# kaspanet/rusty-kaspa

Hardware: NVIDIA H100
Metric: schnorr_sig_verifies_per_sec (higher is better)
Workload: dtype u32 limbs (256-bit modular integer)

## Files before the change

__graft_entry__.py:

```python
import os
import subprocess
import sys

ROOT = os.path.dirname(os.path.abspath(__file__))
CSRC = os.path.join(ROOT, "rusty_kaspa_b200", "csrc")
LIB = os.path.join(ROOT, "rusty_kaspa_b200", "libkgv.so")
NVCC_FLAGS = ["-gencode", "arch=compute_90a,code=sm_90a", "-O3", "-lineinfo", "-std=c++17", "-shared", "-Xcompiler", "-fPIC"]


def _newer(target, sources):
    if not os.path.exists(target):
        return True
    t = os.path.getmtime(target)
    return any(os.path.getmtime(s) > t for s in sources)


def _run(cmd, **kw):
    r = subprocess.run(cmd, capture_output=True, text=True, **kw)
    if r.returncode != 0:
        raise RuntimeError("command failed: %s\n%s\n%s" % (" ".join(cmd), r.stdout[-4000:], r.stderr[-4000:]))
    return r


def build():
    srcs = [os.path.join(d, f) for d, _, fs in os.walk(CSRC) for f in fs] + [os.path.join(ROOT, "include", "kgv.h")]
    units = sorted(s for s in srcs if s.endswith(".cu") or s.endswith(".cpp"))
    if _newer(LIB, srcs):
        nvcc = os.environ.get("NVCC", "nvcc")
        _run([nvcc] + NVCC_FLAGS + ["-o", LIB] + units)
    _run(["make", "-C", os.path.join(ROOT, "oracle")])
    hs = os.path.join(ROOT, "tests", "hostsim")
    for name in ("hostsim_arith", "hostsim_secp", "hostsim_comb", "hostsim_joint", "hostsim_joint_record", "hostsim_hash", "hostsim_u3072", "hostsim_script", "hostsim_standard", "hostsim_chain", "hostsim_pow"):
        src, out = os.path.join(hs, name + ".cpp"), os.path.join(hs, "lib" + name + ".so")
        if os.path.exists(src) and _newer(out, [src] + srcs):
            _run(["g++", "-O2", "-std=c++17", "-shared", "-fPIC", "-o", out, src])
    op_src, op_lib = os.path.join(ROOT, "tests", "oracle_pow", "ok_pow.c"), os.path.join(ROOT, "tests", "oracle_pow", "libok_pow.so")
    if _newer(op_lib, [op_src]):
        _run(["gcc", "-O2", "-std=c11", "-fPIC", "-shared", "-pthread", "-o", op_lib, op_src, "-lm"])
    sg_src, sg_lib = os.path.join(ROOT, "tools", "simgen", "kgv_simgen.cpp"), os.path.join(ROOT, "tools", "simgen", "libkgv_simgen.so")
    if os.path.exists(sg_src) and _newer(sg_lib, [sg_src]):
        _run(["g++", "-O2", "-std=c++17", "-shared", "-fPIC", "-o", sg_lib, sg_src])
    for name in ("host_mirror_test", "script_engine_mirror_test"):
        cpp_src, cpp_bin = os.path.join(ROOT, "tests", "cpp", name + ".cpp"), os.path.join(ROOT, "tests", "cpp", name)
        if os.path.exists(cpp_src) and _newer(cpp_bin, [cpp_src, LIB, os.path.join(ROOT, "include", "kgv.hpp"), os.path.join(ROOT, "include", "kgv.h")]):
            _run(["g++", "-O2", "-std=c++17", "-o", cpp_bin, cpp_src, "-L" + os.path.join(ROOT, "rusty_kaspa_b200"), "-l:libkgv.so", "-Wl,-rpath,$ORIGIN/../../rusty_kaspa_b200"])
    sys.path.insert(0, ROOT)
    import rusty_kaspa_b200
    from rusty_kaspa_b200 import _lib
    _lib.load()


def smoke():
    import ctypes
    import numpy as np
    sys.path.insert(0, ROOT)
# ... 56 lines not shown
```

rusty_kaspa_b200/csrc/kgv_internal.h:

```cpp
#pragma once
#include <cuda_runtime.h>
#include <cstdint>
#include <condition_variable>
#include <cstdio>
#include <initializer_list>
#include <memory>
#include <mutex>
#include <string>
#include <thread>
#include <vector>

#ifndef KGV_BLOCK
#define KGV_BLOCK 128
#endif
#ifndef KGV_BLOCKS_PER_SM
#define KGV_BLOCKS_PER_SM 3
#endif

#ifndef KGV_ITEMS
#define KGV_ITEMS 4
#endif

struct kgv_ctx {
  int device = 0;
  cudaStream_t own_stream = nullptr;
  cudaStream_t aux_stream = nullptr;
  cudaEvent_t ev_fork = nullptr, ev_join = nullptr;
  cudaEvent_t ev_time[3] = {};
  cudaEvent_t ev_chunk[32] = {};
  cudaStream_t stream = nullptr;
  uint32_t* gtab = nullptr;
  uint8_t* d_io = nullptr;
  size_t d_io_cap = 0;
  uint8_t* d_in = nullptr;
  size_t d_in_cap = 0;
  uint8_t* d_out = nullptr;
  size_t d_out_cap = 0;
  uint8_t* d_batch = nullptr;
  size_t d_batch_cap = 0;
  struct PrefetchSlot {
// ... 204 lines not shown
```

rusty_kaspa_b200/csrc/kgv_lib.cu:

```cuda
#include "../../include/kgv.h"
#include "kgv_internal.h"
#include "kgv_verify.cuh"
#include "kgv_lanes.cuh"

#include <cuda_runtime.h>
#include <cstdio>
#include <algorithm>
#include <cstring>
#include <mutex>
#include <string>

using namespace kgv;

struct SmemTab {
  uint32_t* base;
  __device__ __forceinline__ void put(int e, int w, uint32_t v) { base[(e * 16 + w) * KGV_BLOCK] = v; }
  __device__ __forceinline__ uint32_t get(int e, int w) const { return base[(e * 16 + w) * KGV_BLOCK]; }
  __device__ __forceinline__ uint4* chunk(int q) const { return reinterpret_cast<uint4*>(base - threadIdx.x) + q * KGV_BLOCK + threadIdx.x; }
};
__device__ __forceinline__ void stage_fetch(SmemTab& tab, int s, const uint32_t* entry) {
#pragma unroll
  for (int c = 0; c < 4; c++) {
    const uint32_t dst = (uint32_t)__cvta_generic_to_shared(tab.chunk(4 * s + c));
    asm volatile("cp.async.cg.shared.global [%0], [%1], 16;" ::"r"(dst), "l"(entry + 4 * c) : "memory");
  }
}
__device__ __forceinline__ void stage_commit(SmemTab&) { asm volatile("cp.async.commit_group;" ::: "memory"); }
__device__ __forceinline__ void stage_wait(SmemTab&) { asm volatile("cp.async.wait_group 7;" ::: "memory"); }
__device__ __forceinline__ void stage_get(SmemTab& tab, int s, fe& x, fe& y) {
  const uint4 a = *tab.chunk(4 * s), b = *tab.chunk(4 * s + 1), c = *tab.chunk(4 * s + 2), d = *tab.chunk(4 * s + 3);
  x.v[0] = a.x; x.v[1] = a.y; x.v[2] = a.z; x.v[3] = a.w; x.v[4] = b.x; x.v[5] = b.y; x.v[6] = b.z; x.v[7] = b.w;
  y.v[0] = c.x; y.v[1] = c.y; y.v[2] = c.z; y.v[3] = c.w; y.v[4] = d.x; y.v[5] = d.y; y.v[6] = d.z; y.v[7] = d.w;
}

__device__ __forceinline__ void ldg256(uint32_t* w, const void* p) {
  asm volatile("ld.global.nc.v4.u32 {%0,%1,%2,%3}, [%8];\n\t"
               "ld.global.nc.v4.u32 {%4,%5,%6,%7}, [%8+16];"
               : "=r"(w[0]), "=r"(w[1]), "=r"(w[2]), "=r"(w[3]), "=r"(w[4]), "=r"(w[5]), "=r"(w[6]), "=r"(w[7])
               : "l"(p));
}
__device__ __forceinline__ void ldg256_stream(uint32_t* w, const void* p) {
  asm volatile("ld.global.nc.L1::no_allocate.v4.u32 {%0,%1,%2,%3}, [%8];\n\t"
               "ld.global.nc.L1::no_allocate.v4.u32 {%4,%5,%6,%7}, [%8+16];"
               : "=r"(w[0]), "=r"(w[1]), "=r"(w[2]), "=r"(w[3]), "=r"(w[4]), "=r"(w[5]), "=r"(w[6]), "=r"(w[7])
               : "l"(p));
}

struct GLoadDev {
  __device__ __forceinline__ void operator()(fe& x, fe& y, const uint32_t* entry) const {
    ldg256(x.v, entry);
    ldg256(y.v, entry + 8);
  }
};

template <bool ALIGNED>
__device__ __forceinline__ void load_be32(uint32_t* w, const uint8_t* p) {
  if (ALIGNED) {
    ldg256_stream(w, p);
#pragma unroll
    for (int i = 0; i < 8; i++) w[i] = bswap32(w[i]);
  } else {
#pragma unroll
    for (int i = 0; i < 8; i++)
      w[i] = ((uint32_t)p[4 * i] << 24) | ((uint32_t)p[4 * i + 1] << 16) | ((uint32_t)p[4 * i + 2] << 8) | (uint32_t)p[4 * i + 3];
  }
}

__global__ void __launch_bounds__(128) k_build_gtab(uint32_t* __restrict__ gtab) {
  uint32_t t = blockIdx.x * blockDim.x + threadIdx.x;
  if (t >= 8u * 65536u) return;
  uint32_t v = t & 0xFFFFu;
  uint32_t which = t >> 16;
  uint32_t* out = gtab + (size_t)t * 16;
  if (v == 0) {
#pragma unroll
    for (int i = 0; i < 16; i++) out[i] = 0;
    return;
  }
  fe bx, by, x, y;
  gtab_base(bx, by, (int)which);
  gtab_entry(x, y, v, bx, by);
#pragma unroll
  for (int i = 0; i < 8; i++) { out[i] = x.v[i]; out[8 + i] = y.v[i]; }
}

#define KGV_KEY_RECORDS_MAX (1u << 17)
#ifndef KGV_COMB_USES
#define KGV_COMB_USES 8
#endif
enum { KGV_KEYS_INLINE = 0, KGV_KEYS_PLAIN = 1, KGV_KEYS_COMB = 2 };
__host__ __device__ __forceinline__ int key_form(uint32_t n_rec, size_t n) {
  if (n_rec > KGV_KEY_RECORDS_MAX || 2 * (size_t)n_rec > n) return KGV_KEYS_INLINE;
  return (size_t)KGV_COMB_USES * n_rec <= n ? KGV_KEYS_COMB : KGV_KEYS_PLAIN;
}

struct KeySlot {
  unsigned long long key;
  uint32_t rec, unused_;
};
struct KeyCacheView {
  const KeySlot* table;
  const uint32_t* item_slot;
  const uint32_t* recs;
  const uint32_t* n_rec;
  const uint32_t* item_rec;
  const uint32_t* kc_recs;
// ... 481 lines not shown
  if (rc) return rc;
  *cap = want;
  return KGV_OK;
}

extern "C" int kgv_create(int device, uint32_t flags, kgv_ctx** out) {
  (void)flags;
  if (!out) return KGV_ERR_ARG;
  *out = nullptr;
  int ndev = 0;
  if (cudaGetDeviceCount(&ndev) != cudaSuccess || ndev <= 0 || device < 0 || device >= ndev) {
    (void)cudaGetLastError();
    return KGV_ERR_CUDA;
  }
  kgv_ctx* ctx = new kgv_ctx();
  ctx->device = device;
  auto body = [&]() -> int {
    CK(cudaSetDevice(device));
    CK(cudaStreamCreateWithFlags(&ctx->own_stream, cudaStreamNonBlocking));
    ctx->stream = ctx->own_stream;
    CK(cudaStreamCreateWithFlags(&ctx->aux_stream, cudaStreamNonBlocking));
    CK(cudaEventCreateWithFlags(&ctx->ev_fork, cudaEventDisableTiming));
    CK(cudaEventCreateWithFlags(&ctx->ev_join, cudaEventDisableTiming));
    CK(cudaMalloc((void**)&ctx->gtab, (size_t)8 * 65536 * 16 * sizeof(uint32_t)));
    k_build_gtab<<<(8 * 65536) / 128, 128, 0, ctx->stream>>>(ctx->gtab);
    CK(cudaGetLastError());
    ctx->launches++;
    const int smem = KGV_BLOCK * 128 * (int)sizeof(uint32_t);
    for (const auto& kind : k_verify)
      for (const auto& form : kind)
        for (VerifyKernel k : form) CK(cudaFuncSetAttribute(k, cudaFuncAttributeMaxDynamicSharedMemorySize, smem));
    int per_sm = 0, sms = 0;
    CK(cudaOccupancyMaxActiveBlocksPerMultiprocessor(&per_sm, k_verify[0][0][1], KGV_BLOCK, smem));
    CK(cudaDeviceGetAttribute(&sms, cudaDevAttrMultiProcessorCount, device));
    ctx->resident_blocks = per_sm * sms > 0 ? per_sm * sms : 132 * KGV_BLOCKS_PER_SM;
    CK(cudaStreamSynchronize(ctx->stream));
    return KGV_OK;
  };
  int rc = body();
  if (rc != KGV_OK) {
    fprintf(stderr, "kgv_create: %s\n", ctx->err.c_str());
    delete ctx;
    return rc;
  }
  *out = ctx;
  return KGV_OK;
}

extern "C" void kgv_destroy(kgv_ctx* ctx) {
  if (!ctx) return;
  cudaSetDevice(ctx->device);
// ... 146 lines not shown
    P.stamp = 2;
  }
  CK(cudaMemsetAsync(S, 0, 256, st));
  return KGV_OK;
}
static int kc_insert(kgv_ctx* ctx, kgv_keycache::Part& P, const KcScratch& s, size_t n, bool ecdsa, cudaStream_t st, bool gate) {
  CK(cudaMemsetAsync(s.table, 0, (size_t)s.slots * sizeof(KeySlot), st));
  const uint32_t slots = P.v.n_sets * KGV_KC_WAYS, limit = gate ? std::min(slots, (uint32_t)KGV_KEY_RECORDS_MAX) : 0xFFFFFFFFu;
  const auto dedup = ecdsa ? k_key_dedup<false, true, true> : k_key_dedup<true, false, true>;
  dedup<<<nblk(n, 256), 256, 0, st>>>(s.miss_keys, n, nullptr, s.hdr + KC_N_MISS, s.table, s.slots - 1, s.item_slot, s.rec_rep, s.hdr + KC_N_REC,
                                      limit);
  CK(cudaGetLastError());
  const auto insert = ecdsa ? k_kc_insert<true> : k_kc_insert<false>;
  insert<<<nblk(n, KGV_BLOCK), KGV_BLOCK, 0, st>>>(P.v, s.miss_keys, s.rec_rep, s.hdr, P.stamp, gate);
  CK(cudaGetLastError());
  ctx->launches += 2;
  return KGV_OK;
}

int kgv_launch_verify(kgv_ctx* ctx, const uint8_t* dpk, const uint8_t* dmsg, const uint8_t* dsig, size_t n, uint8_t* dst, bool ecdsa,
                      cudaStream_t st, const uint32_t* index, const uint32_t* n_dev) {
  if (n == 0) return KGV_OK;
  if (n >= 0x7FFFFFFFu) return fail_arg(ctx, "verify launch of 2^31 or more items");
  const int smem = KGV_BLOCK * 128 * (int)sizeof(uint32_t);
  size_t want = (n + KGV_BLOCK - 1) / KGV_BLOCK;
  unsigned blocks = (unsigned)(want < (size_t)ctx->resident_blocks ? want : (size_t)ctx->resident_blocks);
  bool aligned = (((uintptr_t)dmsg | (uintptr_t)dsig | (ecdsa ? 0 : (uintptr_t)dpk)) & 31) == 0;
  KeyCacheView kc{};
  const bool key_cache = n > (size_t)ctx->resident_blocks * KGV_BLOCK;
  kgv_keycache::Part* kp = ctx->keycache && ctx->keycache->enabled && ctx->keycache->part[ecdsa].v.n_sets ? &ctx->keycache->part[ecdsa] : nullptr;
  if (!index) {
    auto& lv = ctx->last_verify[ecdsa];
    lv.n = n; lv.blocks = blocks; lv.key_cache = key_cache && !kp; lv.stream = st;
  }
  if (!kp) {
    if (key_cache) {
      int rc = key_cache_launch(ctx, dpk, n, ecdsa, aligned, st, index, n_dev, &kc);
      if (rc) return rc;
    }
    k_verify[ecdsa][index != nullptr][aligned]<<<blocks, KGV_BLOCK, smem, st>>>(dpk, dmsg, dsig, n, dst, ctx->gtab, index, n_dev, kc);
    CK(cudaGetLastError());
    ctx->launches++;
    return KGV_OK;
  }
  KcScratch ks{};
  if (int rc = kc_begin(ctx, *kp, n, ecdsa, st, &ks)) return rc;
  const auto lookup = ecdsa ? k_kc_lookup<false, true> : aligned ? k_kc_lookup<true, false> : k_kc_lookup<false, false>;
// ... 188 lines not shown
  io.out(bitmap, nbytes, &ddst);
  if (int rc = io.stage()) return rc;
  k_status_to_bitmap<<<(unsigned)((nbytes + 255) / 256), 256, 0, ctx->stream>>>(dsrc, n, ddst);
  CK(cudaGetLastError());
  ctx->launches++;
  return io.finish();
}

extern "C" int kgv_debug_schnorr_trace(kgv_ctx* ctx, const uint8_t* pk32, const uint8_t* msg32, const uint8_t* sig64, uint32_t* trace_words,
                                       uint8_t* status) {
  if (!ctx) return KGV_ERR_ARG;
  std::lock_guard<std::recursive_mutex> g(ctx->mu);
  if (!pk32 || !msg32 || !sig64 || !trace_words || !status) return fail_arg(ctx, "null buffer");
  CK(cudaSetDevice(ctx->device));
  const size_t tw = KGV_TRACE_STAGES * 16 * sizeof(uint32_t);
  int rc = kgv_reserve(ctx, &ctx->d_in, &ctx->d_in_cap, 256);
  if (rc) return rc;
  rc = kgv_reserve(ctx, &ctx->d_out, &ctx->d_out_cap, tw + 256);
  if (rc) return rc;
  CK(cudaMemcpyAsync(ctx->d_in, pk32, 32, cudaMemcpyHostToDevice, ctx->stream));
  CK(cudaMemcpyAsync(ctx->d_in + 32, msg32, 32, cudaMemcpyHostToDevice, ctx->stream));
  CK(cudaMemcpyAsync(ctx->d_in + 64, sig64, 64, cudaMemcpyHostToDevice, ctx->stream));
  CK(cudaMemsetAsync(ctx->d_out, 0, tw + 256, ctx->stream));
  const int smem = KGV_BLOCK * 128 * (int)sizeof(uint32_t);
  CK(cudaFuncSetAttribute(k_schnorr_trace, cudaFuncAttributeMaxDynamicSharedMemorySize, smem));
  k_schnorr_trace<<<1, KGV_BLOCK, smem, ctx->stream>>>(ctx->d_in, ctx->d_in + 32, ctx->d_in + 64, ctx->d_out + tw, ctx->gtab, (uint32_t*)ctx->d_out);
  CK(cudaGetLastError());
  ctx->launches++;
  CK(cudaMemcpyAsync(trace_words, ctx->d_out, tw, cudaMemcpyDeviceToHost, ctx->stream));
  CK(cudaMemcpyAsync(status, ctx->d_out + tw, 1, cudaMemcpyDeviceToHost, ctx->stream));
  CK(cudaStreamSynchronize(ctx->stream));
  return KGV_OK;
}

extern "C" int kgv_debug_key_form(kgv_ctx* ctx, int ecdsa, kgv_key_form_info* out) {
  if (!ctx) return KGV_ERR_ARG;
  std::lock_guard<std::recursive_mutex> g(ctx->mu);
  if (!out) return fail_arg(ctx, "null buffer");
  const auto& lv = ctx->last_verify[ecdsa ? 1 : 0];
  if (lv.n == 0) return fail_arg(ctx, "no verify launch of that kind yet");
  CK(cudaSetDevice(ctx->device));
  CK(cudaStreamSynchronize(lv.stream));
  uint32_t n_rec = 0;
  if (lv.key_cache) CK(cudaMemcpy(&n_rec, ctx->d_keys[ecdsa ? 1 : 0], sizeof n_rec, cudaMemcpyDeviceToHost));
  out->n_items = lv.n;
  out->threads = (uint64_t)lv.blocks * KGV_BLOCK;
  out->distinct_keys = n_rec;
// ... 9 lines not shown
  if (!ctx) return KGV_ERR_ARG;
  std::lock_guard<std::recursive_mutex> g(ctx->mu);
  if (!in_words || !out_words || n == 0 || n > (1u << 20)) return fail_arg(ctx, "bad selftest arguments");
  CK(cudaSetDevice(ctx->device));
  int rc = kgv_reserve(ctx, &ctx->d_in, &ctx->d_in_cap, n * 64);
  if (rc) return rc;
  rc = kgv_reserve(ctx, &ctx->d_out, &ctx->d_out_cap, n * 64);
  if (rc) return rc;
  CK(cudaMemcpyAsync(ctx->d_in, in_words, n * 64, cudaMemcpyHostToDevice, ctx->stream));
  if (op >= 12)
    k_selftest_lanes<<<(unsigned)((n * 8 + 63) / 64), 64, 0, ctx->stream>>>(op, (const uint32_t*)ctx->d_in, (uint32_t*)ctx->d_out, (int)n);
  else
    k_selftest<<<(unsigned)((n + 63) / 64), 64, 0, ctx->stream>>>(op, (const uint32_t*)ctx->d_in, (uint32_t*)ctx->d_out, (int)n);
  CK(cudaGetLastError());
  ctx->launches++;
  CK(cudaMemcpyAsync(out_words, ctx->d_out, n * 64, cudaMemcpyDeviceToHost, ctx->stream));
  CK(cudaStreamSynchronize(ctx->stream));
  return KGV_OK;
}

extern "C" int kgv_gtable_entry(kgv_ctx* ctx, int which, uint32_t v, uint8_t out_xy[64]) {
  if (!ctx) return KGV_ERR_ARG;
  std::lock_guard<std::recursive_mutex> g(ctx->mu);
  if ((which != 0 && which != 1) || v == 0 || v > 65535 || !out_xy) return fail_arg(ctx, "bad table index");
  CK(cudaSetDevice(ctx->device));
  uint32_t w[16];
  CK(cudaMemcpyAsync(w, ctx->gtab + ((size_t)which * 4 * 65536 + v) * 16, sizeof w, cudaMemcpyDeviceToHost, ctx->stream));
  CK(cudaStreamSynchronize(ctx->stream));
  for (int c = 0; c < 2; c++)
    for (int i = 0; i < 8; i++) {
      uint32_t limb = w[c * 8 + 7 - i];
      out_xy[c * 32 + 4 * i] = (uint8_t)(limb >> 24);
      out_xy[c * 32 + 4 * i + 1] = (uint8_t)(limb >> 16);
      out_xy[c * 32 + 4 * i + 2] = (uint8_t)(limb >> 8);
      out_xy[c * 32 + 4 * i + 3] = (uint8_t)limb;
    }
  return KGV_OK;
}
```

rusty_kaspa_b200/csrc/kgv_secp.cuh:

```cuda
#pragma once
#include "kgv_arith.cuh"

namespace kgv {

#define KGV_N_LIMBS {0xD0364141u, 0xBFD25E8Cu, 0xAF48A03Bu, 0xBAAEDCE6u, 0xFFFFFFFEu, 0xFFFFFFFFu, 0xFFFFFFFFu, 0xFFFFFFFFu}
#define KGV_BETA_LIMBS {0x719501EEu, 0xC1396C28u, 0x12F58995u, 0x9CF04975u, 0xAC3434E9u, 0x6E64479Eu, 0x657C0710u, 0x7AE96A2Bu}
#define KGV_G1_LIMBS {0x45DBB031u, 0xE893209Au, 0x71E8CA7Fu, 0x3DAA8A14u, 0x9284EB15u, 0xE86C90E4u, 0xA7D46BCDu, 0x3086D221u}
#define KGV_G2_LIMBS {0x8AC47F71u, 0x1571B4AEu, 0x9DF506C6u, 0x221208ACu, 0x0ABFE4C4u, 0x6F547FA9u, 0x010E8828u, 0xE4437ED6u}
#define KGV_A1_LIMBS {0x9284EB15u, 0xE86C90E4u, 0xA7D46BCDu, 0x3086D221u, 0u}
#define KGV_MB1_LIMBS {0x0ABFE4C3u, 0x6F547FA9u, 0x010E8828u, 0xE4437ED6u, 0u}
#define KGV_A2_LIMBS {0x9D44CFD8u, 0x57C1108Du, 0xA8E2F3F6u, 0x14CA50F7u, 1u}

struct gej {
  fe x, y, z;
  bool inf;
};

struct NoTrace {
  KGV_HD void operator()(int , const uint32_t* , int ) const {}
};

KGV_HD bool sc_ge_n(const uint32_t* a) {
  const uint32_t n[8] = KGV_N_LIMBS;
  return !lt8(a, n);
// ... 338 lines not shown
  if (gej_add_ge_body(r, bx, by, hout)) {
    if (hout) fe_dbl(*hout, r.y);
    gej_double_n(r, 1);
  }
}
#endif
KGV_HD void gej_double(gej& r) { gej_double_n(r, 1); }

KGV_HD bool ge_lift_x(fe& y, const fe& x, bool odd) {
  fe t, c;
  fe_sqr(t, x);
  fe_mul(t, t, x);
  fe_set_u32(c, 7);
  fe_add(c, t, c);
  if (!fe_sqrt(y, c)) return false;
  fe_normalize(y);
  if (((y.v[0] & 1u) != 0) != odd) {
    fe_neg(y, y);
    fe_normalize(y);
  }
  return true;
}

template <int NE = 8, class Tab>
KGV_HD void build_odd_table(Tab& tab, fe& zs, const fe& px, const fe& py) {
  static_assert(NE >= 2 && NE <= 8, "build_odd_table: 2 to 8 entries");
  gej d;
  d.x = px; d.y = py; fe_set_u32(d.z, 1); d.inf = false;
  gej_double(d);
  fe zd2, zd3;
  fe_sqr(zd2, d.z);
  fe_mul(zd3, zd2, d.z);
  gej t;
  fe_mul(t.x, px, zd2);
  fe_mul(t.y, py, zd3);
  fe_set_u32(t.z, 1);
  t.inf = false;
  fe H[NE - 1];
#pragma unroll
  for (int w = 0; w < 8; w++) { tab.put(0, w, t.x.v[w]); tab.put(0, 8 + w, t.y.v[w]); }
#pragma unroll
  for (int j = 1; j < NE; j++) {
    gej_add_ge(t, d.x, d.y, &H[j - 1]);
#pragma unroll
    for (int w = 0; w < 8; w++) { tab.put(j, w, t.x.v[w]); tab.put(j, 8 + w, t.y.v[w]); }
  }
// ... 143 lines not shown
      stage_commit(tab);
    }
    if ((w & 3) == 0) {
#pragma unroll 1
      for (int j = 0; j < 8; j++) {
        const uint32_t d = (kG[j] >> (w ? 16 : 0)) & 0xFFFFu;
        if (d) {
          gload(ex, ey, gtab + ((size_t)j * 65536 + d) * 16);
          gej_add_ge(R, ex, ey);
        }
      }
    }
  }
#pragma unroll 1
  for (int half = 0; half < 2; half++) {
    if (!fix[half]) continue;
    gload(ex, ey, rec);
    if (half) fe_mul(ex, ex, beta);
    if (!ng[half]) fe_neg(ey, ey);
    gej_add_ge(R, ex, ey);
  }
}

KGV_HD void recode_joint(uint32_t* h, bool& fix, const uint32_t* m) {
  fix = (m[0] & 1u) == 0;
  uint64_t v[4], carry = fix ? 1 : 0;
#pragma unroll
  for (int t = 0; t < 3; t++) {
    const uint64_t x = (uint64_t)m[t] + carry;
    const uint32_t lo = (uint32_t)x, hi = (uint32_t)(x >> 32);
    const uint32_t borrow = ((m[t + 1] + hi) & 1u) ^ 1u;
    v[t] = (uint64_t)(lo >> 1) + (borrow ? (1ull << 31) : (1ull << 32));
    carry = hi + borrow;
  }
  const uint64_t c3 = (uint64_t)m[3] + ((uint64_t)m[4] << 32) + carry;
  v[3] = (c3 >> 1) + (1ull << 32);
#pragma unroll
  for (int q = 0; q < 5; q++) h[q] = 0;
#pragma unroll
  for (int i = 0; i < 44; i++) h[i / 10] |= (uint32_t)((v[i / 11] >> (3 * (i % 11))) & 7u) << (3 * (i % 10));
}
KGV_HD uint32_t joint_digit(const uint32_t* h, int i) { return (h[i / 10] >> (3 * (i % 10))) & 7u; }
KGV_HD const uint32_t* joint_entry(const uint32_t* jt, const uint32_t (*h)[5], const bool* ng, int i, bool& neg) {
  const uint32_t u0 = joint_digit(h[0], i), u1 = joint_digit(h[1], i);
  neg = (u0 < 4u) != ng[0];
  const uint32_t a = u0 < 4u ? 3u - u0 : u0 - 4u;
  const uint32_t k = neg != ng[1] ? 7u - u1 : u1;
  return jt + 16 * (32 * (i / 11) + 8 * a + k);
}
template <class GLoad>
KGV_HD void gen_fields(gej& R, const uint32_t* kG, int sh, const uint32_t* gtab, GLoad gload) {
  fe ex, ey;
#pragma unroll 1
  for (int j = 0; j < 8; j++) {
    const uint32_t d = (kG[j] >> sh) & 0xFFFFu;
    if (d) {
      gload(ex, ey, gtab + ((size_t)j * 65536 + d) * 16);
      gej_add_ge(R, ex, ey);
    }
  }
}
template <class Tab, class GLoad>
KGV_HD void ecmult_joint(gej& R, const uint32_t* kP, const uint32_t* kG, const uint32_t* rec, const uint32_t* jt, Tab& tab, const uint32_t* gtab,
                         GLoad gload) {
  const fe beta = {KGV_BETA_LIMBS};
  uint32_t m[2][5], h[2][5];
  bool ng[2], fix[2], neg;
  glv_split(m[0], ng[0], m[1], ng[1], kP);
  recode_joint(h[0], fix[0], m[0]);
  recode_joint(h[1], fix[1], m[1]);
#pragma unroll 1
  for (int s = 0; s < 8; s++) {
    const int w = 9 - (s >> 2), t = s & 3;
    stage_fetch(tab, 4 * (w & 1) + t, joint_entry(jt, h, ng, 11 * t + w, neg));
    stage_commit(tab);
  }
  R.inf = true;
  fe_set_zero(R.x); fe_set_zero(R.y); fe_set_zero(R.z);
  fe ex, ey;
#pragma unroll 1
  for (int t = 0; t < 4; t++) {
    gload(ex, ey, joint_entry(jt, h, ng, 11 * t + 10, neg));
    if (neg) fe_neg(ey, ey);
    gej_add_ge(R, ex, ey);
  }
#pragma unroll 1
  for (int w = 9; w >= 0; w--) {
    if (w == 5) {
      gej_double_n(R, 2);
      gen_fields(R, kG, 16, gtab, gload);
      gej_double_n(R, 1);
    } else {
      gej_double_n(R, 3);
    }
#pragma unroll 1
    for (int t = 0; t < 4; t++) {
      const int s = 4 * (w & 1) + t;
      (void)joint_entry(jt, h, ng, 11 * t + w, neg);
      stage_wait(tab);
      stage_get(tab, s, ex, ey);
      if (neg) fe_neg(ey, ey);
      gej_add_ge(R, ex, ey);
      bool neg2;
      if (w >= 2) stage_fetch(tab, s, joint_entry(jt, h, ng, 11 * t + w - 2, neg2));
      stage_commit(tab);
    }
  }
  gen_fields(R, kG, 0, gtab, gload);
  if (fix[0] && fix[1]) {
    gload(ex, ey, jt + 16 * (ng[0] == ng[1] ? 4 : 3));
    if (!ng[0]) fe_neg(ey, ey);
    gej_add_ge(R, ex, ey);
  } else if (fix[0] || fix[1]) {
    const int half = fix[1] ? 1 : 0;
    gload(ex, ey, rec);
    if (half) fe_mul(ex, ex, beta);
    if (!ng[half]) fe_neg(ey, ey);
    gej_add_ge(R, ex, ey);
  }
}

}
```

rusty_kaspa_b200/csrc/kgv_verify.cuh:

```cuda
#pragma once
#include "kgv_secp.cuh"
#include "kgv_sha256.cuh"

namespace kgv {

enum : uint8_t { KGV_ST_INVALID = 0, KGV_ST_VALID = 1, KGV_ST_PK_PARSE = 2, KGV_ST_SIG_PARSE = 3 };

KGV_HD bool fe_words_lt_p(const uint32_t* v) {
  const uint32_t p[8] = {KGV_P0, KGV_P1, 0xFFFFFFFFu, 0xFFFFFFFFu, 0xFFFFFFFFu, 0xFFFFFFFFu, 0xFFFFFFFFu, 0xFFFFFFFFu};
  return lt8(v, p);
}

#define KGV_ST_PENDING 0xFFu

KGV_HD bool key_lift(fe& x, fe& y, uint32_t tag, const uint32_t* pkw) {
  if (tag != 2u && tag != 3u) return false;
  limbs_from_be_words(x.v, pkw);
  if (!fe_words_lt_p(x.v)) return false;
  return ge_lift_x(y, x, tag == 3u);
}

#define KGV_KR_ZS 128
#define KGV_KR_STATUS 136
#define KGV_KR_WORDS 140
// ... 393 lines not shown
  for (int i = 0; i < 8; i++) rf.v[i] = r[i];
  fe_mul(t, rf, zt2);
  if (fe_equal(t, R.x)) return KGV_ST_VALID;
  const uint32_t n[8] = KGV_N_LIMBS;
  uint32_t rn[8];
  uint32_t c = add8(rn, r, n);
  if (c || !fe_words_lt_p(rn)) return KGV_ST_INVALID;
#pragma unroll
  for (int i = 0; i < 8; i++) rf.v[i] = rn[i];
  fe_mul(t, rf, zt2);
  return fe_equal(t, R.x) ? KGV_ST_VALID : KGV_ST_INVALID;
}
template <class Tab, class GLoad>
KGV_HD uint8_t ecdsa_verify_core(uint32_t tag, const uint32_t* pkw, const uint32_t* mw, const uint32_t* sigw, Tab& tab,
                                 const uint32_t* gtab, GLoad gload, KeySrc key = KeySrc{nullptr, false}) {
  fe qx, qy;
  uint32_t r[8], s[8], m[8], sn[8];
  uint8_t st = ecdsa_phase1(qx, qy, r, s, m, tag, pkw, mw, sigw, key);
  if (st != KGV_ST_PENDING) return st;
  sc_inv(sn, s);
  return ecdsa_phase2(qx, qy, r, sn, m, tab, gtab, gload, key);
}

KGV_HD void gtab_entry(fe& ox, fe& oy, uint32_t v, const fe& bx, const fe& by) {
  gej r;
  r.inf = true;
  fe_set_zero(r.x); fe_set_zero(r.y); fe_set_zero(r.z);
  for (int bit = 15; bit >= 0; bit--) {
    gej_double(r);
    if ((v >> bit) & 1u) gej_add_ge(r, bx, by);
  }
  fe zi, zi2;
  fe_inv(zi, r.z);
  fe_sqr(zi2, zi);
  fe_mul(ox, r.x, zi2);
  fe_mul(oy, r.y, zi2);
  fe_mul(oy, oy, zi);
  fe_normalize(ox);
  fe_normalize(oy);
}

#define KGV_GX_LIMBS {0x16F81798u, 0x59F2815Bu, 0x2DCE28D9u, 0x029BFCDBu, 0xCE870B07u, 0x55A06295u, 0xF9DCBBACu, 0x79BE667Eu}
#define KGV_GY_LIMBS {0xFB10D4B8u, 0x9C47D08Fu, 0xA6855419u, 0xFD17B448u, 0x0E1108A8u, 0x5DA4FBFCu, 0x26A3C465u, 0x483ADA77u}
#define KGV_G128X_LIMBS {0x9EC4C0DAu, 0x1B7B444Cu, 0x723EA335u, 0xE88C5678u, 0x981F162Eu, 0x9239C1ADu, 0xF63B5F33u, 0x8F68B9D2u}
#define KGV_G128Y_LIMBS {0x501FFF82u, 0xF23CBF79u, 0x95510BFDu, 0xBBEA2CFEu, 0xB6BE215Du, 0xDE1D90C2u, 0xBA063986u, 0x662A9F2Du}
#define KGV_G32X_LIMBS {0x39A48DB0u, 0xEFD7835Bu, 0x9B3C03BFu, 0x9F1215A2u, 0x9B7BDE45u, 0x2791D0A0u, 0x696E7167u, 0x100F44DAu}
#define KGV_G32Y_LIMBS {0x2BC65A09u, 0x0FBD5CD6u, 0xFF5195ACu, 0xB7FF4A18u, 0x0C090666u, 0x2EC8F330u, 0x92A00B77u, 0xCDD9E131u}
#define KGV_G64X_LIMBS {0x42D0E6BDu, 0x13B7E0E7u, 0xDB0F5E53u, 0xF774D163u, 0x104D6ECBu, 0x82A2147Cu, 0x243C4E25u, 0x3322D401u}
#define KGV_G64Y_LIMBS {0x6C28B2A0u, 0x24F3A2E9u, 0xA2873AF6u, 0x2805F63Eu, 0x4DDAF9B7u, 0xBFB019BCu, 0xE9664EF5u, 0x56E70797u}
#define KGV_G96X_LIMBS {0x40FB27B6u, 0x32427E28u, 0xBE430576u, 0xC76E3DB2u, 0x61686AA5u, 0x10F238ADu, 0xBE778B1Bu, 0xFEA74E3Du}
#define KGV_G96Y_LIMBS {0xF23CB96Fu, 0x701D3DB7u, 0x973F7B77u, 0x126B596Bu, 0xCCB6AF93u, 0x7CF674DEu, 0x9B0B1329u, 0x6E0568DBu}
#define KGV_G160X_LIMBS {0xAC1F98CDu, 0xCBFC99C8u, 0x4D7F0308u, 0x52348905u, 0x1CC66021u, 0xFAED8A9Cu, 0x4A474870u, 0x9C3919A8u}
#define KGV_G160Y_LIMBS {0xD4FC599Du, 0xBE7E5E03u, 0x6C64C8E6u, 0x905326F7u, 0xF260E641u, 0x584F044Bu, 0x4A4DDD57u, 0xDDB84F0Fu}
#define KGV_G192X_LIMBS {0x2120E2B3u, 0x7F3B58FAu, 0x7F47F9AAu, 0x7A58FDCEu, 0x4CE6E521u, 0xE7BE4AE3u, 0x1F51BDBAu, 0xEAA649F2u}
#define KGV_G192Y_LIMBS {0xBA5AD93Du, 0xD47A5305u, 0xF13F7E59u, 0x01A6B965u, 0x9879AA5Au, 0xC69A80F8u, 0x5BBBB03Au, 0xBE3279EDu}
#define KGV_G224X_LIMBS {0x9475B7BAu, 0x884FDFF0u, 0xE4918B3Du, 0xE039E730u, 0xF5018CDBu, 0x3D3E57EDu, 0x1943785Cu, 0x95939698u}
#define KGV_G224Y_LIMBS {0x7524F2FDu, 0xE9B8ABF8u, 0xC8709385u, 0x9C653F64u, 0x4B9CD684u, 0x8BA0386Au, 0x88C331DDu, 0x2E7E5528u}
KGV_HD void gtab_base(fe& x, fe& y, int j) {
  const fe bx[8] = {{KGV_GX_LIMBS}, {KGV_G32X_LIMBS}, {KGV_G64X_LIMBS}, {KGV_G96X_LIMBS}, {KGV_G128X_LIMBS}, {KGV_G160X_LIMBS}, {KGV_G192X_LIMBS}, {KGV_G224X_LIMBS}};
  const fe by[8] = {{KGV_GY_LIMBS}, {KGV_G32Y_LIMBS}, {KGV_G64Y_LIMBS}, {KGV_G96Y_LIMBS}, {KGV_G128Y_LIMBS}, {KGV_G160Y_LIMBS}, {KGV_G192Y_LIMBS}, {KGV_G224Y_LIMBS}};
  x = bx[j];
  y = by[j];
}

}
```

Baseline: 64.66 million.

## Replace generator 16-bit windowed fields with signed-digit comb table interleaved into joint loop

Replaces the 16 generator-table additions (two gen_fields passes over eight 16-bit windows) with a signed-digit 8-tooth comb. It uses a new 2^23-entry precomputed table built at context init, giving 11 generator additions spread through the joint ecmult loop. Comb entries are prefetched into shared memory via cp.async one window ahead, so the shared table per thread grows from 128 to 144 words. This cuts point additions and hides gather latency, at the cost of a large extra device table (about 512 MB), higher init time and possibly lower occupancy.

```diff
diff --git a/__graft_entry__.py b/__graft_entry__.py
--- a/__graft_entry__.py
+++ b/__graft_entry__.py
@@ -30,7 +30,7 @@
         _run([nvcc] + NVCC_FLAGS + ["-o", LIB] + units)
     _run(["make", "-C", os.path.join(ROOT, "oracle")])
     hs = os.path.join(ROOT, "tests", "hostsim")
-    for name in ("hostsim_arith", "hostsim_secp", "hostsim_comb", "hostsim_joint", "hostsim_joint_record", "hostsim_hash", "hostsim_u3072", "hostsim_script", "hostsim_standard", "hostsim_chain", "hostsim_pow"):
+    for name in ("hostsim_arith", "hostsim_secp", "hostsim_comb", "hostsim_joint", "hostsim_joint_record", "hostsim_gen_comb", "hostsim_hash", "hostsim_u3072", "hostsim_script", "hostsim_standard", "hostsim_chain", "hostsim_pow"):
         src, out = os.path.join(hs, name + ".cpp"), os.path.join(hs, "lib" + name + ".so")
         if os.path.exists(src) and _newer(out, [src] + srcs):
             _run(["g++", "-O2", "-std=c++17", "-shared", "-fPIC", "-o", out, src])
diff --git a/rusty_kaspa_b200/csrc/kgv_internal.h b/rusty_kaspa_b200/csrc/kgv_internal.h
--- a/rusty_kaspa_b200/csrc/kgv_internal.h
+++ b/rusty_kaspa_b200/csrc/kgv_internal.h
@@ -16,6 +16,7 @@
 #ifndef KGV_BLOCKS_PER_SM
 #define KGV_BLOCKS_PER_SM 3
 #endif
+#define KGV_TAB_WORDS 144
 
 #ifndef KGV_ITEMS
 #define KGV_ITEMS 4
diff --git a/rusty_kaspa_b200/csrc/kgv_lib.cu b/rusty_kaspa_b200/csrc/kgv_lib.cu
--- a/rusty_kaspa_b200/csrc/kgv_lib.cu
+++ b/rusty_kaspa_b200/csrc/kgv_lib.cu
@@ -32,6 +32,14 @@
   x.v[0] = a.x; x.v[1] = a.y; x.v[2] = a.z; x.v[3] = a.w; x.v[4] = b.x; x.v[5] = b.y; x.v[6] = b.z; x.v[7] = b.w;
   y.v[0] = c.x; y.v[1] = c.y; y.v[2] = c.z; y.v[3] = c.w; y.v[4] = d.x; y.v[5] = d.y; y.v[6] = d.z; y.v[7] = d.w;
 }
+__device__ __forceinline__ void gen_fetch(SmemTab& tab, const uint32_t* gtab, uint32_t u) {
+  stage_fetch(tab, 8, gtab + KGV_GC_OFF + (size_t)u * 16);
+}
+__device__ __forceinline__ void gen_get(SmemTab& tab, const uint32_t*, uint32_t, bool first, fe& x, fe& y) {
+  if (first) asm volatile("cp.async.wait_group 7;" ::: "memory");
+  else asm volatile("cp.async.wait_group 3;" ::: "memory");
+  stage_get(tab, 8, x, y);
+}
 
 __device__ __forceinline__ void ldg256(uint32_t* w, const void* p) {
   asm volatile("ld.global.nc.v4.u32 {%0,%1,%2,%3}, [%8];\n\t"
@@ -52,7 +60,6 @@
     ldg256(y.v, entry + 8);
   }
 };
-
 template <bool ALIGNED>
 __device__ __forceinline__ void load_be32(uint32_t* w, const uint8_t* p) {
   if (ALIGNED) {
@@ -82,6 +89,58 @@
   gtab_entry(x, y, v, bx, by);
 #pragma unroll
   for (int i = 0; i < 8; i++) { out[i] = x.v[i]; out[8 + i] = y.v[i]; }
+}
+
+__global__ void __launch_bounds__(128) k_build_gcomb(uint32_t* __restrict__ gtab) {
+  const uint32_t V = blockIdx.x * blockDim.x + threadIdx.x;
+  if (V >= KGV_GC_ENTRIES / 4) return;
+  const uint32_t u0 = 4 * V;
+  gej q;
+  q.inf = true;
+  fe_set_zero(q.x); fe_set_zero(q.y); fe_set_zero(q.z);
+  fe x, y;
+#pragma unroll 1
+  for (int j = 7; j >= 1; j--) {
+    const int d = gc_digit(u0, j);
+    const uint32_t* e = gtab + ((size_t)j * 65536 + (uint32_t)(d < 0 ? -d : d)) * 16;
+    fe_ld(x, e);
+    fe_ld(y, e + 8);
+    if (d < 0) fe_neg(y, y);
+    gej_add_ge(q, x, y);
+  }
+  gej r[4];
+  fe pre[4];
+#pragma unroll 1
+  for (int a = 0; a < 4; a++) {
+    const uint32_t* e = gtab + (size_t)(2 * a + 1) * 16;
+    fe_ld(x, e);
+    fe_ld(y, e + 8);
+    r[a] = q;
+    gej_add_ge(r[a], x, y);
+    if (a) fe_mul(pre[a], pre[a - 1], r[a].z);
+    else pre[0] = r[0].z;
+  }
+  fe inv;
+  fe_inv(inv, pre[3]);
+#pragma unroll 1
+  for (int a = 3; a >= 0; a--) {
+    fe zi, zi2;
+    if (a) {
+      fe_mul(zi, inv, pre[a - 1]);
+      fe_mul(inv, inv, r[a].z);
+    } else {
+      zi = inv;
+    }
+    fe_sqr(zi2, zi);
+    fe_mul(x, r[a].x, zi2);
+    fe_mul(y, r[a].y, zi2);
+    fe_mul(y, y, zi);
+    fe_normalize(x);
+    fe_normalize(y);
+    uint32_t* out = gtab + KGV_GC_OFF + (size_t)(u0 + a) * 16;
+    fe_st(out, x);
+    fe_st(out + 8, y);
+  }
 }
 
 #define KGV_KEY_RECORDS_MAX (1u << 17)
@@ -609,11 +668,13 @@
     CK(cudaStreamCreateWithFlags(&ctx->aux_stream, cudaStreamNonBlocking));
     CK(cudaEventCreateWithFlags(&ctx->ev_fork, cudaEventDisableTiming));
     CK(cudaEventCreateWithFlags(&ctx->ev_join, cudaEventDisableTiming));
-    CK(cudaMalloc((void**)&ctx->gtab, (size_t)8 * 65536 * 16 * sizeof(uint32_t)));
+    CK(cudaMalloc((void**)&ctx->gtab, (KGV_GC_OFF + (size_t)KGV_GC_ENTRIES * 16) * sizeof(uint32_t)));
     k_build_gtab<<<(8 * 65536) / 128, 128, 0, ctx->stream>>>(ctx->gtab);
     CK(cudaGetLastError());
-    ctx->launches++;
-    const int smem = KGV_BLOCK * 128 * (int)sizeof(uint32_t);
+    k_build_gcomb<<<KGV_GC_ENTRIES / 4 / 128, 128, 0, ctx->stream>>>(ctx->gtab);
+    CK(cudaGetLastError());
+    ctx->launches += 2;
+    const int smem = KGV_BLOCK * KGV_TAB_WORDS * (int)sizeof(uint32_t);
     for (const auto& kind : k_verify)
       for (const auto& form : kind)
         for (VerifyKernel k : form) CK(cudaFuncSetAttribute(k, cudaFuncAttributeMaxDynamicSharedMemorySize, smem));
@@ -806,7 +867,7 @@
                       cudaStream_t st, const uint32_t* index, const uint32_t* n_dev) {
   if (n == 0) return KGV_OK;
   if (n >= 0x7FFFFFFFu) return fail_arg(ctx, "verify launch of 2^31 or more items");
-  const int smem = KGV_BLOCK * 128 * (int)sizeof(uint32_t);
+  const int smem = KGV_BLOCK * KGV_TAB_WORDS * (int)sizeof(uint32_t);
   size_t want = (n + KGV_BLOCK - 1) / KGV_BLOCK;
   unsigned blocks = (unsigned)(want < (size_t)ctx->resident_blocks ? want : (size_t)ctx->resident_blocks);
   bool aligned = (((uintptr_t)dmsg | (uintptr_t)dsig | (ecdsa ? 0 : (uintptr_t)dpk)) & 31) == 0;
@@ -1041,7 +1102,7 @@
   CK(cudaMemcpyAsync(ctx->d_in + 32, msg32, 32, cudaMemcpyHostToDevice, ctx->stream));
   CK(cudaMemcpyAsync(ctx->d_in + 64, sig64, 64, cudaMemcpyHostToDevice, ctx->stream));
   CK(cudaMemsetAsync(ctx->d_out, 0, tw + 256, ctx->stream));
-  const int smem = KGV_BLOCK * 128 * (int)sizeof(uint32_t);
+  const int smem = KGV_BLOCK * KGV_TAB_WORDS * (int)sizeof(uint32_t);
   CK(cudaFuncSetAttribute(k_schnorr_trace, cudaFuncAttributeMaxDynamicSharedMemorySize, smem));
   k_schnorr_trace<<<1, KGV_BLOCK, smem, ctx->stream>>>(ctx->d_in, ctx->d_in + 32, ctx->d_in + 64, ctx->d_out + tw, ctx->gtab, (uint32_t*)ctx->d_out);
   CK(cudaGetLastError());
@@ -1097,10 +1158,12 @@
 extern "C" int kgv_gtable_entry(kgv_ctx* ctx, int which, uint32_t v, uint8_t out_xy[64]) {
   if (!ctx) return KGV_ERR_ARG;
   std::lock_guard<std::recursive_mutex> g(ctx->mu);
-  if ((which != 0 && which != 1) || v == 0 || v > 65535 || !out_xy) return fail_arg(ctx, "bad table index");
+  if (which < 0 || which > 2 || (which < 2 && (v == 0 || v > 65535)) || (which == 2 && v >= KGV_GC_ENTRIES) || !out_xy)
+    return fail_arg(ctx, "bad table index");
   CK(cudaSetDevice(ctx->device));
   uint32_t w[16];
-  CK(cudaMemcpyAsync(w, ctx->gtab + ((size_t)which * 4 * 65536 + v) * 16, sizeof w, cudaMemcpyDeviceToHost, ctx->stream));
+  const size_t e = which == 2 ? KGV_GC_OFF + (size_t)v * 16 : ((size_t)which * 4 * 65536 + v) * 16;
+  CK(cudaMemcpyAsync(w, ctx->gtab + e, sizeof w, cudaMemcpyDeviceToHost, ctx->stream));
   CK(cudaStreamSynchronize(ctx->stream));
   for (int c = 0; c < 2; c++)
     for (int i = 0; i < 8; i++) {
diff --git a/rusty_kaspa_b200/csrc/kgv_secp.cuh b/rusty_kaspa_b200/csrc/kgv_secp.cuh
--- a/rusty_kaspa_b200/csrc/kgv_secp.cuh
+++ b/rusty_kaspa_b200/csrc/kgv_secp.cuh
@@ -384,6 +384,72 @@
   return true;
 }
 
+KGV_HD void gtab_entry(fe& ox, fe& oy, uint32_t v, const fe& bx, const fe& by) {
+  gej r;
+  r.inf = true;
+  fe_set_zero(r.x); fe_set_zero(r.y); fe_set_zero(r.z);
+  for (int bit = 15; bit >= 0; bit--) {
+    gej_double(r);
+    if ((v >> bit) & 1u) gej_add_ge(r, bx, by);
+  }
+  fe zi, zi2;
+  fe_inv(zi, r.z);
+  fe_sqr(zi2, zi);
+  fe_mul(ox, r.x, zi2);
+  fe_mul(oy, r.y, zi2);
+  fe_mul(oy, oy, zi);
+  fe_normalize(ox);
+  fe_normalize(oy);
+}
+
+#define KGV_GX_LIMBS {0x16F81798u, 0x59F2815Bu, 0x2DCE28D9u, 0x029BFCDBu, 0xCE870B07u, 0x55A06295u, 0xF9DCBBACu, 0x79BE667Eu}
+#define KGV_GY_LIMBS {0xFB10D4B8u, 0x9C47D08Fu, 0xA6855419u, 0xFD17B448u, 0x0E1108A8u, 0x5DA4FBFCu, 0x26A3C465u, 0x483ADA77u}
+#define KGV_G128X_LIMBS {0x9EC4C0DAu, 0x1B7B444Cu, 0x723EA335u, 0xE88C5678u, 0x981F162Eu, 0x9239C1ADu, 0xF63B5F33u, 0x8F68B9D2u}
+#define KGV_G128Y_LIMBS {0x501FFF82u, 0xF23CBF79u, 0x95510BFDu, 0xBBEA2CFEu, 0xB6BE215Du, 0xDE1D90C2u, 0xBA063986u, 0x662A9F2Du}
+#define KGV_G32X_LIMBS {0x39A48DB0u, 0xEFD7835Bu, 0x9B3C03BFu, 0x9F1215A2u, 0x9B7BDE45u, 0x2791D0A0u, 0x696E7167u, 0x100F44DAu}
+#define KGV_G32Y_LIMBS {0x2BC65A09u, 0x0FBD5CD6u, 0xFF5195ACu, 0xB7FF4A18u, 0x0C090666u, 0x2EC8F330u, 0x92A00B77u, 0xCDD9E131u}
+#define KGV_G64X_LIMBS {0x42D0E6BDu, 0x13B7E0E7u, 0xDB0F5E53u, 0xF774D163u, 0x104D6ECBu, 0x82A2147Cu, 0x243C4E25u, 0x3322D401u}
+#define KGV_G64Y_LIMBS {0x6C28B2A0u, 0x24F3A2E9u, 0xA2873AF6u, 0x2805F63Eu, 0x4DDAF9B7u, 0xBFB019BCu, 0xE9664EF5u, 0x56E70797u}
+#define KGV_G96X_LIMBS {0x40FB27B6u, 0x32427E28u, 0xBE430576u, 0xC76E3DB2u, 0x61686AA5u, 0x10F238ADu, 0xBE778B1Bu, 0xFEA74E3Du}
+#define KGV_G96Y_LIMBS {0xF23CB96Fu, 0x701D3DB7u, 0x973F7B77u, 0x126B596Bu, 0xCCB6AF93u, 0x7CF674DEu, 0x9B0B1329u, 0x6E0568DBu}
+#define KGV_G160X_LIMBS {0xAC1F98CDu, 0xCBFC99C8u, 0x4D7F0308u, 0x52348905u, 0x1CC66021u, 0xFAED8A9Cu, 0x4A474870u, 0x9C3919A8u}
+#define KGV_G160Y_LIMBS {0xD4FC599Du, 0xBE7E5E03u, 0x6C64C8E6u, 0x905326F7u, 0xF260E641u, 0x584F044Bu, 0x4A4DDD57u, 0xDDB84F0Fu}
+#define KGV_G192X_LIMBS {0x2120E2B3u, 0x7F3B58FAu, 0x7F47F9AAu, 0x7A58FDCEu, 0x4CE6E521u, 0xE7BE4AE3u, 0x1F51BDBAu, 0xEAA649F2u}
+#define KGV_G192Y_LIMBS {0xBA5AD93Du, 0xD47A5305u, 0xF13F7E59u, 0x01A6B965u, 0x9879AA5Au, 0xC69A80F8u, 0x5BBBB03Au, 0xBE3279EDu}
+#define KGV_G224X_LIMBS {0x9475B7BAu, 0x884FDFF0u, 0xE4918B3Du, 0xE039E730u, 0xF5018CDBu, 0x3D3E57EDu, 0x1943785Cu, 0x95939698u}
+#define KGV_G224Y_LIMBS {0x7524F2FDu, 0xE9B8ABF8u, 0xC8709385u, 0x9C653F64u, 0x4B9CD684u, 0x8BA0386Au, 0x88C331DDu, 0x2E7E5528u}
+KGV_HD void gtab_base(fe& x, fe& y, int j) {
+  const fe bx[8] = {{KGV_GX_LIMBS}, {KGV_G32X_LIMBS}, {KGV_G64X_LIMBS}, {KGV_G96X_LIMBS}, {KGV_G128X_LIMBS}, {KGV_G160X_LIMBS}, {KGV_G192X_LIMBS}, {KGV_G224X_LIMBS}};
+  const fe by[8] = {{KGV_GY_LIMBS}, {KGV_G32Y_LIMBS}, {KGV_G64Y_LIMBS}, {KGV_G96Y_LIMBS}, {KGV_G128Y_LIMBS}, {KGV_G160Y_LIMBS}, {KGV_G192Y_LIMBS}, {KGV_G224Y_LIMBS}};
+  x = bx[j];
+  y = by[j];
+}
+
+#define KGV_GC_OFF ((size_t)8 * 65536 * 16)
+#define KGV_GC_ENTRIES (1u << 23)
+KGV_HD int gc_digit(uint32_t u, int j) { return j ? 2 * (int)((u >> (3 * j - 1)) & 7u) - 7 : 2 * (int)(u & 3u) + 1; }
+KGV_HD void gc_entry(fe& ox, fe& oy, uint32_t u) {
+  gej r;
+  r.inf = true;
+  fe_set_zero(r.x); fe_set_zero(r.y); fe_set_zero(r.z);
+  for (int j = 0; j < 8; j++) {
+    const int d = gc_digit(u, j);
+    fe bx, by, x, y;
+    gtab_base(bx, by, j);
+    gtab_entry(x, y, (uint32_t)(d < 0 ? -d : d), bx, by);
+    if (d < 0) fe_neg(y, y);
+    gej_add_ge(r, x, y);
+  }
+  fe zi, zi2;
+  fe_inv(zi, r.z);
+  fe_sqr(zi2, zi);
+  fe_mul(ox, r.x, zi2);
+  fe_mul(oy, r.y, zi2);
+  fe_mul(oy, oy, zi);
+  fe_normalize(ox);
+  fe_normalize(oy);
+}
+
 template <int NE = 8, class Tab>
 KGV_HD void build_odd_table(Tab& tab, fe& zs, const fe& px, const fe& py) {
   static_assert(NE >= 2 && NE <= 8, "build_odd_table: 2 to 8 entries");
@@ -573,17 +639,19 @@
   }
 }
 
+KGV_HD uint64_t joint_tooth(uint32_t mt, uint32_t mn, uint32_t& carry) {
+  const uint64_t x = (uint64_t)mt + carry;
+  const uint32_t lo = (uint32_t)x, hi = (uint32_t)(x >> 32);
+  const uint32_t borrow = ((mn + hi) & 1u) ^ 1u;
+  carry = hi + borrow;
+  return (uint64_t)(lo >> 1) + (borrow ? (1ull << 31) : (1ull << 32));
+}
 KGV_HD void recode_joint(uint32_t* h, bool& fix, const uint32_t* m) {
   fix = (m[0] & 1u) == 0;
-  uint64_t v[4], carry = fix ? 1 : 0;
-#pragma unroll
-  for (int t = 0; t < 3; t++) {
-    const uint64_t x = (uint64_t)m[t] + carry;
-    const uint32_t lo = (uint32_t)x, hi = (uint32_t)(x >> 32);
-    const uint32_t borrow = ((m[t + 1] + hi) & 1u) ^ 1u;
-    v[t] = (uint64_t)(lo >> 1) + (borrow ? (1ull << 31) : (1ull << 32));
-    carry = hi + borrow;
-  }
+  uint64_t v[4];
+  uint32_t carry = fix ? 1 : 0;
+#pragma unroll
+  for (int t = 0; t < 3; t++) v[t] = joint_tooth(m[t], m[t + 1], carry);
   const uint64_t c3 = (uint64_t)m[3] + ((uint64_t)m[4] << 32) + carry;
   v[3] = (c3 >> 1) + (1ull << 32);
 #pragma unroll
@@ -599,24 +667,53 @@
   const uint32_t k = neg != ng[1] ? 7u - u1 : u1;
   return jt + 16 * (32 * (i / 11) + 8 * a + k);
 }
-template <class GLoad>
-KGV_HD void gen_fields(gej& R, const uint32_t* kG, int sh, const uint32_t* gtab, GLoad gload) {
-  fe ex, ey;
-#pragma unroll 1
-  for (int j = 0; j < 8; j++) {
-    const uint32_t d = (kG[j] >> sh) & 0xFFFFu;
-    if (d) {
-      gload(ex, ey, gtab + ((size_t)j * 65536 + d) * 16);
-      gej_add_ge(R, ex, ey);
+KGV_HD void recode_gen(uint32_t* h, bool& neg, const uint32_t* s) {
+  const uint32_t n[8] = KGV_N_LIMBS;
+  uint32_t r[8];
+  neg = (s[0] & 1u) == 0;
+  if (neg) (void)sub8(r, n, s);
+#pragma unroll
+  for (int i = 0; i < 8; i++) r[i] = neg ? r[i] : s[i];
+  uint64_t v[8];
+  uint32_t carry = 0;
+#pragma unroll
+  for (int j = 0; j < 7; j++) v[j] = joint_tooth(r[j], r[j + 1], carry);
+  v[7] = (((uint64_t)r[7] + carry) >> 1) + (1ull << 32);
+#pragma unroll
+  for (int q = 0; q < 9; q++) h[q] = 0;
+#pragma unroll
+  for (int w = 0; w < 11; w++) {
+#pragma unroll
+    for (int j = 0; j < 8; j++) {
+      const int b = 24 * w + 3 * j;
+      const uint32_t f = (uint32_t)(v[j] >> (3 * w)) & 7u;
+      h[b >> 5] |= f << (b & 31);
+      if ((b & 31) > 29) h[(b >> 5) + 1] |= f >> (32 - (b & 31));
     }
   }
+}
+KGV_HD uint32_t gen_entry(const uint32_t* h, int w, bool& neg) {
+  const int b = 24 * w;
+  const uint64_t x = (uint64_t)h[b >> 5] | ((uint64_t)h[(b >> 5) + 1] << 32);
+  uint32_t f = (uint32_t)(x >> (b & 31)) & 0xFFFFFFu;
+  neg = (f & 4u) == 0;
+  if (neg) f ^= 0xFFFFFFu;
+  return (f & 3u) | ((f >> 1) & ~3u);
+}
+template <class Tab>
+KGV_HD void gen_fetch(Tab&, const uint32_t*, uint32_t) {}
+template <class Tab>
+KGV_HD void gen_get(Tab&, const uint32_t*, uint32_t u, bool, fe& x, fe& y) {
+  gc_entry(x, y, u);
 }
 template <class Tab, class GLoad>
 KGV_HD void ecmult_joint(gej& R, const uint32_t* kP, const uint32_t* kG, const uint32_t* rec, const uint32_t* jt, Tab& tab, const uint32_t* gtab,
                          GLoad gload) {
   const fe beta = {KGV_BETA_LIMBS};
-  uint32_t m[2][5], h[2][5];
-  bool ng[2], fix[2], neg;
+  uint32_t m[2][5], h[2][5], hg[9];
+  bool ng[2], fix[2], gneg, neg;
+  recode_gen(hg, gneg, kG);
+  gen_fetch(tab, gtab, gen_entry(hg, 10, neg));
   glv_split(m[0], ng[0], m[1], ng[1], kP);
   recode_joint(h[0], fix[0], m[0]);
   recode_joint(h[1], fix[1], m[1]);
@@ -636,28 +733,27 @@
     gej_add_ge(R, ex, ey);
   }
 #pragma unroll 1
-  for (int w = 9; w >= 0; w--) {
-    if (w == 5) {
-      gej_double_n(R, 2);
-      gen_fields(R, kG, 16, gtab, gload);
-      gej_double_n(R, 1);
-    } else {
+  for (int w = 10; w >= 0; w--) {
+    if (w < 10) {
       gej_double_n(R, 3);
+#pragma unroll 1
+      for (int t = 0; t < 4; t++) {
+        const int s = 4 * (w & 1) + t;
+        (void)joint_entry(jt, h, ng, 11 * t + w, neg);
+        stage_wait(tab);
+        stage_get(tab, s, ex, ey);
+        if (neg) fe_neg(ey, ey);
+        gej_add_ge(R, ex, ey);
+        bool neg2;
+        if (w >= 2) stage_fetch(tab, s, joint_entry(jt, h, ng, 11 * t + w - 2, neg2));
+        stage_commit(tab);
+      }
     }
-#pragma unroll 1
-    for (int t = 0; t < 4; t++) {
-      const int s = 4 * (w & 1) + t;
-      (void)joint_entry(jt, h, ng, 11 * t + w, neg);
-      stage_wait(tab);
-      stage_get(tab, s, ex, ey);
-      if (neg) fe_neg(ey, ey);
-      gej_add_ge(R, ex, ey);
-      bool neg2;
-      if (w >= 2) stage_fetch(tab, s, joint_entry(jt, h, ng, 11 * t + w - 2, neg2));
-      stage_commit(tab);
-    }
-  }
-  gen_fields(R, kG, 0, gtab, gload);
+    gen_get(tab, gtab, gen_entry(hg, w, neg), w == 10, ex, ey);
+    if (neg != gneg) fe_neg(ey, ey);
+    gej_add_ge(R, ex, ey);
+    if (w) gen_fetch(tab, gtab, gen_entry(hg, w - 1, neg));
+  }
   if (fix[0] && fix[1]) {
     gload(ex, ey, jt + 16 * (ng[0] == ng[1] ? 4 : 3));
     if (!ng[0]) fe_neg(ey, ey);
diff --git a/rusty_kaspa_b200/csrc/kgv_verify.cuh b/rusty_kaspa_b200/csrc/kgv_verify.cuh
--- a/rusty_kaspa_b200/csrc/kgv_verify.cuh
+++ b/rusty_kaspa_b200/csrc/kgv_verify.cuh
@@ -439,45 +439,4 @@
   return ecdsa_phase2(qx, qy, r, sn, m, tab, gtab, gload, key);
 }
 
-KGV_HD void gtab_entry(fe& ox, fe& oy, uint32_t v, const fe& bx, const fe& by) {
-  gej r;
-  r.inf = true;
-  fe_set_zero(r.x); fe_set_zero(r.y); fe_set_zero(r.z);
-  for (int bit = 15; bit >= 0; bit--) {
-    gej_double(r);
-    if ((v >> bit) & 1u) gej_add_ge(r, bx, by);
-  }
-  fe zi, zi2;
-  fe_inv(zi, r.z);
-  fe_sqr(zi2, zi);
-  fe_mul(ox, r.x, zi2);
-  fe_mul(oy, r.y, zi2);
-  fe_mul(oy, oy, zi);
-  fe_normalize(ox);
-  fe_normalize(oy);
-}
-
-#define KGV_GX_LIMBS {0x16F81798u, 0x59F2815Bu, 0x2DCE28D9u, 0x029BFCDBu, 0xCE870B07u, 0x55A06295u, 0xF9DCBBACu, 0x79BE667Eu}
-#define KGV_GY_LIMBS {0xFB10D4B8u, 0x9C47D08Fu, 0xA6855419u, 0xFD17B448u, 0x0E1108A8u, 0x5DA4FBFCu, 0x26A3C465u, 0x483ADA77u}
-#define KGV_G128X_LIMBS {0x9EC4C0DAu, 0x1B7B444Cu, 0x723EA335u, 0xE88C5678u, 0x981F162Eu, 0x9239C1ADu, 0xF63B5F33u, 0x8F68B9D2u}
-#define KGV_G128Y_LIMBS {0x501FFF82u, 0xF23CBF79u, 0x95510BFDu, 0xBBEA2CFEu, 0xB6BE215Du, 0xDE1D90C2u, 0xBA063986u, 0x662A9F2Du}
-#define KGV_G32X_LIMBS {0x39A48DB0u, 0xEFD7835Bu, 0x9B3C03BFu, 0x9F1215A2u, 0x9B7BDE45u, 0x2791D0A0u, 0x696E7167u, 0x100F44DAu}
-#define KGV_G32Y_LIMBS {0x2BC65A09u, 0x0FBD5CD6u, 0xFF5195ACu, 0xB7FF4A18u, 0x0C090666u, 0x2EC8F330u, 0x92A00B77u, 0xCDD9E131u}
-#define KGV_G64X_LIMBS {0x42D0E6BDu, 0x13B7E0E7u, 0xDB0F5E53u, 0xF774D163u, 0x104D6ECBu, 0x82A2147Cu, 0x243C4E25u, 0x3322D401u}
-#define KGV_G64Y_LIMBS {0x6C28B2A0u, 0x24F3A2E9u, 0xA2873AF6u, 0x2805F63Eu, 0x4DDAF9B7u, 0xBFB019BCu, 0xE9664EF5u, 0x56E70797u}
-#define KGV_G96X_LIMBS {0x40FB27B6u, 0x32427E28u, 0xBE430576u, 0xC76E3DB2u, 0x61686AA5u, 0x10F238ADu, 0xBE778B1Bu, 0xFEA74E3Du}
-#define KGV_G96Y_LIMBS {0xF23CB96Fu, 0x701D3DB7u, 0x973F7B77u, 0x126B596Bu, 0xCCB6AF93u, 0x7CF674DEu, 0x9B0B1329u, 0x6E0568DBu}
-#define KGV_G160X_LIMBS {0xAC1F98CDu, 0xCBFC99C8u, 0x4D7F0308u, 0x52348905u, 0x1CC66021u, 0xFAED8A9Cu, 0x4A474870u, 0x9C3919A8u}
-#define KGV_G160Y_LIMBS {0xD4FC599Du, 0xBE7E5E03u, 0x6C64C8E6u, 0x905326F7u, 0xF260E641u, 0x584F044Bu, 0x4A4DDD57u, 0xDDB84F0Fu}
-#define KGV_G192X_LIMBS {0x2120E2B3u, 0x7F3B58FAu, 0x7F47F9AAu, 0x7A58FDCEu, 0x4CE6E521u, 0xE7BE4AE3u, 0x1F51BDBAu, 0xEAA649F2u}
-#define KGV_G192Y_LIMBS {0xBA5AD93Du, 0xD47A5305u, 0xF13F7E59u, 0x01A6B965u, 0x9879AA5Au, 0xC69A80F8u, 0x5BBBB03Au, 0xBE3279EDu}
-#define KGV_G224X_LIMBS {0x9475B7BAu, 0x884FDFF0u, 0xE4918B3Du, 0xE039E730u, 0xF5018CDBu, 0x3D3E57EDu, 0x1943785Cu, 0x95939698u}
-#define KGV_G224Y_LIMBS {0x7524F2FDu, 0xE9B8ABF8u, 0xC8709385u, 0x9C653F64u, 0x4B9CD684u, 0x8BA0386Au, 0x88C331DDu, 0x2E7E5528u}
-KGV_HD void gtab_base(fe& x, fe& y, int j) {
-  const fe bx[8] = {{KGV_GX_LIMBS}, {KGV_G32X_LIMBS}, {KGV_G64X_LIMBS}, {KGV_G96X_LIMBS}, {KGV_G128X_LIMBS}, {KGV_G160X_LIMBS}, {KGV_G192X_LIMBS}, {KGV_G224X_LIMBS}};
-  const fe by[8] = {{KGV_GY_LIMBS}, {KGV_G32Y_LIMBS}, {KGV_G64Y_LIMBS}, {KGV_G96Y_LIMBS}, {KGV_G128Y_LIMBS}, {KGV_G160Y_LIMBS}, {KGV_G192Y_LIMBS}, {KGV_G224Y_LIMBS}};
-  x = bx[j];
-  y = by[j];
-}
-
-}
+}
```

Measured after the change: 67.01 million (median of 6 runs). 3.6% higher.
